# xiaohong-huang/RTK-Visual-Inertial-Navigation

Hardware: AMD Instinct MI355X
Metric: gauss_newton_iterations_per_sec (higher is better)
Workload: dtype f64; 1 GPU; BASELINE cfg4: batch of 512 independent cfg3 windows (20 keyframes, 300 features, 3000 observations, 19 IMU factors, 10 satellites x 20 epochs carrier-phase+pseudorange, gauge prior) over the job, 8 dogleg iterations per solve; windows=512, windows_rank0=512

## Files before the change

### rtk_visual_inertial_navigation_amd/build.py

```python
import os
import subprocess

HERE = os.path.dirname(os.path.abspath(__file__))
CSRC = os.path.join(HERE, "csrc")
LIB = os.path.join(HERE, "libswf_hip.so")
SOURCES = ["swf_engine.hip", "swf_plan.cpp", "swf_problem.cpp", "swf_producers.hip", "swf_gnss_epochs.cpp", "swf_lambda.hip", "swf_features.hip", "swf_fixprior.hip", "swf_phasescreen.hip", "swf_gnssepoch.hip", "swf_ddselect.hip"]
HEADERS = ["swf_dev.h", "swf_records.h", "swf_plan.h", "swf_kernels.h", "swf_lmschur.h", "swf_chol_rr4.h", "swf_kernels2.h", "swf_kernels3.h", "swf_rootdev.h", "swf_kernels4.h", "swf_lambda.h", "swf_features.h", "swf_fixprior.h", "swf_gnss_range.h", "swf_phasescreen.h", "swf_gnssepoch.h", "swf_ddselect.h",
           os.path.join("..", "..", "include", "swf_types.h"),
           os.path.join("..", "..", "include", "swf_solver.h")]


def hipcc():
    for p in (os.environ.get("HIPCC"), "/opt/rocm/bin/hipcc", "hipcc"):
        if p and (os.path.isabs(p) and os.path.exists(p) or not os.path.isabs(p)):
            return p
    return "hipcc"


def needs_build():
    if not os.path.exists(LIB):
        return True
    t = os.path.getmtime(LIB)
    for f in SOURCES + HEADERS:
        p = os.path.join(CSRC, f)
        if os.path.exists(p) and os.path.getmtime(p) > t:
            return True
    return False


def build(force=False, verbose=False):
    if not force and not needs_build():
        return LIB
    srcs = [os.path.join(CSRC, s) for s in SOURCES if os.path.exists(os.path.join(CSRC, s))]
    cmd = [hipcc(), "--offload-arch=gfx950", "-O3", "-std=c++17", "-fPIC", "-shared"] + \
        os.environ.get("SWF_EXTRA_FLAGS", "").split() + ["-x", "hip", "-o", LIB] + srcs
    if verbose:
        print(" ".join(cmd))
    subprocess.check_call(cmd, cwd=CSRC)
    return LIB


if __name__ == "__main__":
    print(build(force=True, verbose=True))
```

### rtk_visual_inertial_navigation_amd/csrc/swf_engine.hip

```cpp
#include <hip/hip_runtime.h>
#include <algorithm>
#include <chrono>
#include <cmath>
#include <cstdio>
#include <cstdlib>
#include <cstring>
#include <string>
#include <memory>
#include <thread>
#include <vector>
#include "../../include/swf_solver.h"
#include "swf_kernels2.h"
#include "swf_kernels3.h"
#include "swf_kernels4.h"
#include "swf_lambda.h"
#include "swf_ddselect.h"
#include "swf_features.h"
#include "swf_fixprior.h"
#include "swf_plan.h"

static thread_local std::string g_err;
static int fail(int code, const std::string& msg) { g_err = msg; return code; }
#define HIPCHK(x) do { hipError_t e_ = (x); if (e_ != hipSuccess) return fail(SWF_E_NODEVICE, std::string(#x) + ": " + hipGetErrorString(e_)); } while (0)

// ... 155 lines not shown
    DevPool pool;
    hipStream_t stream = nullptr;
    std::vector<WinRec> win;
    std::vector<HostWin> hw;
    int max_tiles = 0, max_prior_dim = 0, max_red = 0, min_red = 1 << 30, n_cu = 256;
    bool clc_imu[5] = { false, false, false, false, false };
    CompArgs CA{}; CompMeta CM{}; int n_comp = 0, comp_nmax = 0, comp_nmin = 1 << 30; long long comp_ne = 0;
    bool comp_eigen_root = false;
    void* h_sum = nullptr; size_t h_sum_bytes = 0;
    double* h_x = nullptr;
    double* co_pose0 = nullptr; double* co_sb0 = nullptr;
    int* mg_tail = nullptr; double* mg_A = nullptr; double* mg_b = nullptr; double* mg_J = nullptr; double* mg_r0 = nullptr; double* mg_w = nullptr; int* mg_rank = nullptr; double* mg_M = nullptr;
    bool mg_valid = false; int mg_ld = 0;
    bool mg_host = false; std::vector<double> h_mgA, h_mgJ, h_mgb, h_mgr0, h_mgw; std::vector<int> h_mgrank;
    double* mg_resM = nullptr; double* mg_resb = nullptr; int* mg_resok = nullptr;
    int* mg_rot = nullptr; int* mg_bjok = nullptr; unsigned long long* mg_crit = nullptr;
    int* tc_tail = nullptr; double* tc_A = nullptr; double* tc_Q = nullptr; double* tc_X = nullptr; int* tc_rank = nullptr; bool tc_valid = false; int tc_ld = 0;
    int* am_first = nullptr; int4* am_pairs = nullptr; double* am_rec = nullptr; int am_rec_ld = 0;
    bool am_valid = false, am_host = false; std::vector<double> h_am;
    std::vector<int> am_nb;
    std::vector<int> am_h_first; std::vector<int4> am_h_pairs;
    int* dd_pairs = nullptr; int* dd_counts = nullptr; int* dd_npair = nullptr;
    char* dd_in = nullptr; char* dd_out = nullptr; size_t dd_in_cap = 0, dd_out_cap = 0; int dd_ne = 0, dd_no = 0;
    std::vector<char> dd_h_in, dd_h_out; std::vector<int> dd_h_pairs, dd_h_counts;
    bool dd_valid = false, dd_host = false;
    const int* dd_tail = nullptr;
    bool am_selected = false, am_sel_host = false;
    FixWin* fx_win = nullptr; int* fx_tailcol = nullptr; double* fx_A = nullptr; double* fx_b = nullptr; double* fx_J = nullptr; double* fx_r0 = nullptr;
    double* fx_eig = nullptr; double* fx_x0 = nullptr; int* fx_rank = nullptr; int* fx_applied = nullptr; int fx_ldn = 0, fx_ldx = 0;
    bool fx_valid = false, fx_host = false; FixPriorArgs fx_args{};
    std::vector<FixWin> fx_h_win; std::vector<int> fx_h_tailcol, fx_sel;
    std::vector<double> h_fxA, h_fxb, h_fxJ, h_fxr0, h_fxeig, h_fxx0; std::vector<int> h_fxrank, h_fxapplied;
    bool fc_built = false, fc_valid = false, fc_host = false; FeatArgs fc{}; char* fc_out = nullptr; size_t fc_bytes = 0; int fc_nfeat = 0;
    std::vector<int> fc_feat0; std::vector<char> h_fc;
    hipStream_t aux = nullptr; hipEvent_t ev_fork[3] = { nullptr, nullptr, nullptr };
    ~swf_batch() {
        if (aux) { (void)hipStreamSynchronize(aux); handle_cache().give(aux); }
        for (auto& e : ev_fork) handle_cache().give(e, false);
    }
    WinState* ws_primary = nullptr; WinState* ws_alt = nullptr; WinState* ws_alt2 = nullptr;
    bool no_decide_fuse = false;
    bool no_step_fuse = false;
    int n_pch_split = 0;
    bool no_spec = false;
    bool no_comp_fuse = false;
    bool lat_fuse = false;
    bool rr4_has15 = false, rr4_has16 = false;
    int rr_nmax = 256;
    bool L_full = false;
    int asm_programs = 0;
    int ls_qpb = 1, ls_var = 0, ls_kms = 8; bool ls_folded = false, s_direct = false;
    bool full_final = false;
    bool no_clq_pack = false;
    int clp_rows = 1, clp_ld = 3;
    int ls_gqpb = 4;
    int timing = 0;
    swf_timing last{};
    std::vector<hipEvent_t> ev;
    std::vector<int> ev_kind;
    int ev_used = 0;
    int64_t jac_bytes = 0, proj_bytes = 0, chol_flops = 0, lm_schur_flops = 0, lm_schur_flops_sym = 0, lm_schur_mfma = 0;
    int last_mode = -1;
};

extern "C" int swf_batch_create(const swf_flat_window* const* windows, int32_t n, void* stream, swf_batch** out) {
    if (!windows || n <= 0 || !out) return fail(SWF_E_INVALID, "swf_batch_create: bad arguments");
    int ndev = 0;
    if (hipGetDeviceCount(&ndev) != hipSuccess || ndev <= 0)
        return fail(SWF_E_NODEVICE, "no HIP device: this library has no CPU fallback");
    int n_cu = 256;
    { int dev = 0; hipDeviceProp_t pr; if (hipGetDevice(&dev) == hipSuccess && hipGetDeviceProperties(&pr, dev) == hipSuccess && pr.multiProcessorCount > 0) n_cu = pr.multiProcessorCount; }
    Plan B;
    {
        std::string err;
        int prc = plan_build(windows, n, plan_shape_from_env(n_cu), B, err);
        if (prc != SWF_OK) return fail(prc, err);
    }
    std::unique_ptr<swf_batch> owner(new swf_batch());
    swf_batch* b = owner.get();
    b->device = current_device();
    b->stream = (hipStream_t)stream;
    b->n_cu = n_cu;
    b->no_comp_fuse = getenv("SWF_NO_COMP_FUSE") != nullptr;
    b->no_spec = getenv("SWF_NO_SPEC_EVAL") != nullptr;
    b->no_step_fuse = getenv("SWF_NO_STEP_FUSE") != nullptr;
    b->no_decide_fuse = getenv("SWF_NO_DECIDE_FUSE") != nullptr;
    b->full_final = getenv("SWF_FULL_FINAL_ELIM") != nullptr;
    b->no_clq_pack = getenv("SWF_NO_CLIQUE_PACK") != nullptr;
    b->max_tiles = B.max_tiles; b->max_prior_dim = B.max_prior_dim; b->max_red = B.max_red; b->min_red = B.min_red;
    b->rr_nmax = B.rr_nmax; b->rr4_has15 = B.rr4_has15; b->rr4_has16 = B.rr4_has16; b->n_pch_split = B.n_pch_split;
    b->lat_fuse = B.lat_fuse; b->asm_programs = B.asm_programs;
    b->ls_qpb = B.ls_qpb; b->ls_var = B.ls_var; b->ls_kms = B.ls_kms; b->ls_gqpb = B.ls_gqpb; b->ls_folded = B.ls_folded; b->s_direct = B.s_direct;
    for (int k = 0; k < 5; k++) b->clc_imu[k] = B.clc_imu[k];
    b->clp_rows = B.clp_rows; b->clp_ld = B.clp_ld;
    b->n_comp = B.n_comp; b->comp_nmax = B.comp_nmax; b->comp_nmin = B.comp_nmin; b->comp_ne = B.comp_ne;
    b->jac_bytes = B.jac_bytes; b->proj_bytes = B.proj_bytes; b->chol_flops = B.chol_flops;
    b->lm_schur_flops = B.lm_schur_flops; b->lm_schur_flops_sym = B.lm_schur_flops_sym; b->lm_schur_mfma = B.lm_schur_mfma;
    if (B.want_aux) {
        bool ok = (b->aux = handle_cache().stream()) != nullptr;
        for (int i = 0; i < 3 && ok; i++) ok = (b->ev_fork[i] = handle_cache().event(false)) != nullptr;
        if (!ok) { handle_cache().give(b->aux); b->aux = nullptr; }
    }
    DevBatch& D = b->D;
    DevPool& P = b->pool;
    int rc = 0;
    D.n_win = n; D.n_x = (int)B.n_x; D.n_loc_total = (int)B.n_loc; D.max_iter_trace = SWF_MAX_TRACE; D.rr_nmax = B.rr_nmax;
    D.n_lmb = B.n_lmb; D.n_pch = B.n_pch; D.n_proj = B.n_proj; D.n_lm = B.n_lm; D.n_fr = B.n_fr; D.n_fsb = B.n_fsb;
    D.n_gf = (int)B.gf.size(); D.n_imu = (int)B.imu_gf.size(); D.n_sc = (int)B.sc_gf.size(); D.n_prior = (int)B.prior_gf.size(); D.n_idp = (int)B.idp_gf.size();
    D.n_cl = (int)B.cl.size(); D.n_pair = (int)B.pair.size(); D.n_pd = B.n_pd; D.n_po = B.n_po; D.n_cle = B.n_cle;
    for (int k = 0; k < 5; k++) D.n_clc[k] = B.n_clc[k];
    D.as_max_ne = B.as_max_ne; D.as_max_nv = B.as_max_nv;
#define PUT(field) rc |= P.put(B.field, &D.field)
    PUT(win);
    PUT(lmb_rec); PUT(pch_q); PUT(pch_r0); PUT(prior_nch);
    PUT(blk_xoff); PUT(blk_loc); PUT(blk_gs);
    PUT(loc2x); PUT(x_var);
    PUT(p_win); PUT(p_xpose); PUT(p_xex); PUT(p_xlm);
    PUT(p_lpose); PUT(p_llm); PUT(p_fr); PUT(p_lm); PUT(p_uv);
    PUT(lm_win); PUT(lm_obs0); PUT(lm_loc); PUT(lm_col); PUT(lm_fmask);
    PUT(sch_c0); PUT(sch_rec); PUT(sch_km);
    PUT(fr_obs0); PUT(fr_obs); PUT(fr_red);
    PUT(fsb_rec);
    PUT(fsb_perm); PUT(fsb_foff);
    PUT(gf);
    PUT(s_x); PUT(s_loc); PUT(s_ls); PUT(s_joff); PUT(s_ccol);
    PUT(imu_pre); PUT(cp_dat); PUT(pr_dat); PUT(dop_dat); PUT(sp_w); PUT(gx_dat);
    PUT(imu_gf); PUT(sc_gf); PUT(prior_gf); PUT(idp_gf);
    PUT(sc_jt); PUT(imu_jt);
    PUT(prior_dim); PUT(prior_Joff); PUT(prior_roff); PUT(prior_x0off);
    PUT(prior_Jt);
    PUT(prior_colloc); PUT(prior_colcc); PUT(s_pcol); PUT(s_pxo);
    PUT(prior_J); PUT(prior_r0); PUT(prior_x0);
    PUT(cl); PUT(cl_fac); PUT(cl_frow); PUT(cm_loc); PUT(cm_ls); PUT(cm_col);
    PUT(cv_loc);
    PUT(pc_coff); PUT(pc_cld); PUT(pc_voff);
    PUT(asw); PUT(s_tnz);
    PUT(as_dst); PUT(as_cnt); PUT(as_src0); PUT(as_aux); PUT(as_src);
    PUT(av_loc); PUT(av_red); PUT(av_cnt); PUT(av_src0); PUT(av_i); PUT(av_src);
    PUT(pair_d); PUT(pair_o);
    PUT(cle_rec);
    for (int k = 0; k < 5; k++) PUT(clc_rec[k]);
// ... 303 lines not shown
        hipStream_t sa = fork ? b->aux : st;
        if (fork) { (void)hipEventRecord(b->ev_fork[0], st); (void)hipStreamWaitEvent(b->aux, b->ev_fork[0], 0); }
        bool imu_fused = false;
        if (D.n_proj + D.n_sc + D.n_prior) {
            Bracket t(*this, SWF_K_EVAL_PS);
            bool pf = b->max_prior_dim <= PRIOR_LDS_DIM;
            Segs S{}; S.e[0] = D.n_fsb; S.e[1] = S.e[0] + nb(D.n_sc, 256); S.e[2] = S.e[1] + (pf ? D.n_pch : 0);
            imu_fused = b->lat_fuse && D.n_imu > 0;
            S.e[3] = S.e[2] + (imu_fused ? nb(D.n_imu, IMU_FPB) : 0);
            if (imu_fused) hipLaunchKernelGGL((k_eval_ps<true, true, true>), dim3(S.e[3]), dim3(256), 0, st, D, S);
            else hipLaunchKernelGGL((k_eval_ps<true, true>), dim3(S.e[2]), dim3(256), 0, st, D, S);
        }
        if (D.n_idp) hipLaunchKernelGGL(k_eval_idp<true>, GRID(D.n_idp, 128), dim3(128), 0, st, D);
        if (D.n_prior && b->max_prior_dim > PRIOR_LDS_DIM) { Bracket t(*this, SWF_K_EVAL_PRIOR); hipLaunchKernelGGL(k_eval_prior<true>, dim3(D.n_pch), dim3(256), (2 * b->max_prior_dim + 16) * sizeof(double), st, D); }
        if (fork) (void)hipEventRecord(b->ev_fork[1], st);
        if (D.n_imu && !imu_fused) { Bracket t(*this, SWF_K_EVAL_IMU, sa); hipLaunchKernelGGL(k_eval_imu<true>, GRID(D.n_imu, IMU_FPB), dim3(IMU_FPB * IMU_LPF), 0, sa, D); }
    }
    void lin_elim(int write_S) {
        DevBatch& D = b->D;
        bool clq_fused = false;
        if (comp_fused) {
            Bracket t(*this, SWF_K_CLIQUE_ELIM);
            if (D.n_clc[3]) {
                hipLaunchKernelGGL(k_clique_big2, dim3(D.n_clc[3] + D.n_clc[2]), dim3(CB_NT), 0, st, D, O);
                if (D.n_clc[4]) hipLaunchKernelGGL(k_clique_tall<false>, dim3(D.n_clc[4]), dim3(256), 0, st, D, O);
            } else if (D.n_clc[4] + D.n_clc[2]) hipLaunchKernelGGL(k_clique_tall2, dim3(D.n_clc[4] + D.n_clc[2]), dim3(256), 0, st, D, O);
        } else if (D.n_lm) {
            Bracket t(*this, write_S ? SWF_K_LM_SCHUR : SWF_K_LM_ELIM);
            lm_qpb = b->ls_qpb; lm_folded = b->ls_folded;
            if (!write_S && !b->full_final) {
                dim3 grid(D.n_win, GEMM_SPLIT / b->ls_gqpb);
                hipLaunchKernelGGL((k_lm_schur<8, 2, 2, 80, false, true>), grid, dim3(256), 0, st, D, O, b->ls_gqpb, 0, 0, 0);
            } else if (!write_S) {
                dim3 grid(D.n_win, GEMM_SPLIT / lm_qpb);
                hipLaunchKernelGGL((k_lm_schur<8, 2, 2, 80, false>), grid, dim3(256), 0, st, D, O, lm_qpb, 0, 0, 0);
            } else {
                const int crow = D.n_win > 0 ? (D.n_clc[2] + D.n_win - 1) / D.n_win : 0;
                clq_fused = clq_fuse_ok();
                lm_launch(0, st, clq_fused ? crow : 0);
                lm_next = ls_tiles_per_launch();
            }
        }
        {
            hipStream_t sa = b->aux ? b->aux : st;
            if (b->aux) (void)hipStreamWaitEvent(b->aux, b->ev_fork[1], 0);
            auto cstream = [&](int cls) { return (b->aux && !b->clc_imu[cls]) ? st : sa; };
            if (comp_fused) {
                for (; lm_next < b->max_tiles; lm_next += ls_tiles_per_launch()) { Bracket t(*this, SWF_K_LM_SCHUR, sa); lm_launch(lm_next, sa); }
            } else {
            const bool grad = !write_S && !b->full_final;
            if (D.n_clc[1]) {
                Bracket t(*this, SWF_K_CLIQUE_ELIM, cstream(1));
                if (grad) hipLaunchKernelGGL((k_clique_elim<32, 48, 9, 1, true>), dim3(D.n_clc[1]), dim3(64), 0, cstream(1), D, O);
                else hipLaunchKernelGGL((k_clique_elim<32, 48, 9, 1>), dim3(D.n_clc[1]), dim3(64), 0, cstream(1), D, O);
            }
            if (D.n_clc[0]) {
                Bracket t(*this, SWF_K_CLIQUE_ELIM, cstream(0));
                constexpr int CLP_NW = 1;
                const size_t lds = CLP_NW * 2 * ((size_t)(b->clp_rows + 2) * b->clp_ld + b->clp_rows + 2) * sizeof(double);
                const dim3 cgrid(((D.n_clc[0] + 1) / 2 + CLP_NW - 1) / CLP_NW);
                if (b->no_clq_pack) {
                    if (grad) hipLaunchKernelGGL((k_clique_elim<48, 32, 1, 0, true>), dim3(D.n_clc[0]), dim3(64), 0, cstream(0), D, O);
                    else hipLaunchKernelGGL((k_clique_elim<48, 32, 1, 0>), dim3(D.n_clc[0]), dim3(64), 0, cstream(0), D, O);
                }
                else if (grad) hipLaunchKernelGGL((k_clique_pack<true, CLP_NW>), cgrid, dim3(64 * CLP_NW), lds, cstream(0), D, O, b->clp_rows, b->clp_ld);
                else hipLaunchKernelGGL((k_clique_pack<false, CLP_NW>), cgrid, dim3(64 * CLP_NW), lds, cstream(0), D, O, b->clp_rows, b->clp_ld);
            }
            if (D.n_clc[2] && !clq_fused) {
                Bracket t(*this, SWF_K_CLIQUE_ELIM, cstream(2));
                if (b->lat_fuse) {
                    if (grad) hipLaunchKernelGGL(k_clique_elim4<true>, dim3(D.n_clc[2]), dim3(256), 0, cstream(2), D, O);
                    else hipLaunchKernelGGL(k_clique_elim4<false>, dim3(D.n_clc[2]), dim3(256), 0, cstream(2), D, O);
                }
                else if (grad) hipLaunchKernelGGL((k_clique_elim<64, 64, 9, 2, true>), dim3(D.n_clc[2]), dim3(64), 0, cstream(2), D, O);
                else hipLaunchKernelGGL((k_clique_elim<64, 64, 9, 2>), dim3(D.n_clc[2]), dim3(64), 0, cstream(2), D, O);
            }
            if (D.n_clc[3]) { Bracket t(*this, SWF_K_CLIQUE_ELIM, cstream(3)); hipLaunchKernelGGL(k_clique_big, dim3(D.n_clc[3]), dim3(CB_NT), 0, cstream(3), D, O); }
            if (D.n_clc[4]) {
                Bracket t(*this, SWF_K_CLIQUE_ELIM, cstream(4));
                if (grad) hipLaunchKernelGGL(k_clique_tall<true>, dim3(D.n_clc[4]), dim3(256), 0, cstream(4), D, O);
                else hipLaunchKernelGGL(k_clique_tall<false>, dim3(D.n_clc[4]), dim3(256), 0, cstream(4), D, O);
            }
            if (write_S && D.n_lm) {
                for (; lm_next < b->max_tiles; lm_next += ls_tiles_per_launch()) { Bracket t(*this, SWF_K_LM_SCHUR, sa); lm_launch(lm_next, sa); }
            }
            }
            if (b->aux) (void)hipEventRecord(b->ev_fork[2], b->aux);
        }
        if (b->n_pch_split) hipLaunchKernelGGL(k_prior_graw, dim3(D.n_pch), dim3(256), 0, st, D);
        if (b->aux) (void)hipStreamWaitEvent(st, b->ev_fork[2], 0);
        if (D.n_pd) {
            Bracket t(*this, SWF_K_ASSEMBLE);
            const int nbS = write_S ? nb((size_t)D.as_max_ne, 256) : 0, nbV = nb((size_t)D.as_max_nv, 256);
            hipLaunchKernelGGL(k_assemble_flat, dim3(nbS + nbV, D.n_win), dim3(256), 0, st, D, O, write_S, nbS);
        }
    }
    void reduced() {
        DevBatch& D = b->D;
        Bracket t(*this, SWF_K_CHOL);
        if (b->max_red <= CB_NMAX) {
            if (b->min_red <= b->rr_nmax) {
                if (b->min_red <= 224) hipLaunchKernelGGL(k_chol_rr4<14>, dim3(D.n_win), dim3(R4_NT), 0, st, D, export_full ? 1 : 0);
                if (b->rr4_has15) hipLaunchKernelGGL(k_chol_rr4<15>, dim3(D.n_win), dim3(R4_NT), 0, st, D, export_full ? 1 : 0);
                if (b->rr4_has16) hipLaunchKernelGGL(k_chol_rr4<16>, dim3(D.n_win), dim3(R4_NT), 0, st, D, export_full ? 1 : 0);
            }
            if (b->max_red > b->rr_nmax && D.Wk) {
                const int Tc = (b->max_red + 15) / 16;
// ... 911 lines not shown
        if (r) ok &= dl(r + row, D.g_r + G.roff, (size_t)G.nres * 8);
        if (J && G.type == GF_PRIOR) {
            int dim = 0; long long jo = 0;
            ok &= dl(&dim, D.prior_dim + G.data, 4); ok &= dl(&jo, D.prior_Joff + G.data, 8);
            std::vector<double> PJ((size_t)dim * dim);
            ok &= dl(PJ.data(), D.prior_J + jo, PJ.size() * 8);
            for (int sl = 0; sl < G.nslot; sl++) {
                if (sloc[sl] < 0) continue;
                for (int k = 0; k < G.nres; k++) for (int c = 0; c < sls[sl]; c++)
                    J[(row + k) * nl + (sloc[sl] - W.loc_base) + c] = PJ[(size_t)k * dim + spc[sl] + c];
            }
        } else if (J) {
            for (int sl = 0; sl < G.nslot; sl++) {
                if (sloc[sl] < 0 || sj[sl] < 0) continue;
                std::vector<double> blk((size_t)sls[sl] * G.jld);
                ok &= dl(blk.data(), D.g_J + sj[sl], (((size_t)sls[sl] - 1) * G.jld + G.nres) * 8);
                for (int k = 0; k < G.nres; k++) for (int c = 0; c < sls[sl]; c++)
                    J[(row + k) * nl + (sloc[sl] - W.loc_base) + c] = blk[(size_t)c * G.jld + k];
            }
        }
        if (G.type != GF_PROJX) row_seq += G.nres;
    }
    if (!ok) return fail(SWF_E_NODEVICE, "download failed");
    return SWF_OK;
}

extern "C" int swf_debug_plan_check(const swf_flat_window* const* windows, int32_t n, int32_t n_cu, int32_t ls_variant, int32_t ls_qpb, int32_t ls_grad_qpb,
                                    int32_t flags, int32_t corrupt_table, int32_t corrupt_index, int32_t* info) {
    if (!windows || n <= 0 || n_cu <= 0) return fail(SWF_E_INVALID, "swf_debug_plan_check: bad arguments");
    PlanShape sh;
    sh.n_cu = n_cu; sh.ls_variant = ls_variant; sh.ls_qpb = ls_qpb; sh.ls_grad_qpb = ls_grad_qpb; sh.no_lat_fuse = flags & 1; sh.no_chol_col = flags & 2;
    Plan B; std::string err;
    int rc = plan_build(windows, n, sh, B, err);
    if (rc != SWF_OK) return fail(rc, err);
    if (corrupt_table) {
        const size_t i = (size_t)corrupt_index;
        if (corrupt_table == 1 && i < B.as_src.size()) B.as_src[i] += 1 << 28;
        else if (corrupt_table == 2 && i < B.sch_rec.size()) B.sch_rec[i] ^= 1;
        else if (corrupt_table == 3 && i < B.s_tnz.size() && B.s_tnz[i]) B.s_tnz[i] &= B.s_tnz[i] - 1;
        else if (corrupt_table == 4 && i < B.prior_colloc.size()) B.prior_colloc[i] ^= 1;
        else if (corrupt_table == 5 && i < B.loc2x.size()) B.loc2x[i] ^= 1;
        else if (corrupt_table == 6 && i < B.co_voff.size()) B.co_voff[i] += 1 << 28;
        else if (corrupt_table == 7 && i < B.pair_o.size()) B.pair_o[i].q_base += 8;
        else return fail(SWF_E_INVALID, "swf_debug_plan_check: nothing to corrupt there");
    }
    if (info) {
        const int v[12] = { B.ls_var, B.ls_qpb, B.ls_gqpb, B.ls_folded, B.lat_fuse, B.want_aux, B.want_Linv, B.want_Wk, B.asm_programs, B.n_pch_split, B.max_red, B.n_pch };
        for (int k = 0; k < 12; k++) info[k] = v[k];
    }
    rc = plan_validate(B, err);
    return rc == SWF_OK ? SWF_OK : fail(rc, err);
}

#ifdef SWF_PROFILE_CHOL
extern "C" int swf_debug_chol_stamps(unsigned long long* out) {
    if (hipDeviceSynchronize() != hipSuccess) return SWF_E_NODEVICE;
    if (hipMemcpyFromSymbol(out, HIP_SYMBOL(g_chol_stamps), 64 * sizeof(unsigned long long)) != hipSuccess) return SWF_E_NODEVICE;
    return SWF_OK;
}
#endif

#ifdef SWF_PROFILE_CHOLW
extern "C" int swf_debug_chol_wstep(int step) {
    if (hipDeviceSynchronize() != hipSuccess) return SWF_E_NODEVICE;
    unsigned long long z[16 * 8] = { 0 };
    if (hipMemcpyToSymbol(HIP_SYMBOL(g_chol_wst), z, sizeof(z)) != hipSuccess) return SWF_E_NODEVICE;
    if (hipMemcpyToSymbol(HIP_SYMBOL(g_chol_wstep), &step, sizeof(int)) != hipSuccess) return SWF_E_NODEVICE;
    return SWF_OK;
}
extern "C" int swf_debug_chol_wstamps(unsigned long long* out) {
    if (hipDeviceSynchronize() != hipSuccess) return SWF_E_NODEVICE;
    if (hipMemcpyFromSymbol(out, HIP_SYMBOL(g_chol_wst), 16 * 8 * sizeof(unsigned long long)) != hipSuccess) return SWF_E_NODEVICE;
    return SWF_OK;
}
extern "C" int swf_debug_chol_pstamps(unsigned long long* out) {
    if (hipDeviceSynchronize() != hipSuccess) return SWF_E_NODEVICE;
    if (hipMemcpyFromSymbol(out, HIP_SYMBOL(g_chol_pst), 16 * sizeof(unsigned long long)) != hipSuccess) return SWF_E_NODEVICE;
    return SWF_OK;
}
extern "C" int swf_debug_chol_cstamps(unsigned long long* out) {
    if (hipDeviceSynchronize() != hipSuccess) return SWF_E_NODEVICE;
    if (hipMemcpyFromSymbol(out, HIP_SYMBOL(g_chol_cst), 32 * sizeof(unsigned long long)) != hipSuccess) return SWF_E_NODEVICE;
    return SWF_OK;
}
#endif

#ifdef SWF_PROFILE_DOG
extern "C" int swf_debug_dog_stamps(unsigned long long* out) {
    if (hipDeviceSynchronize() != hipSuccess) return SWF_E_NODEVICE;
    if (hipMemcpyFromSymbol(out, HIP_SYMBOL(g_dog_stamps), 16 * sizeof(unsigned long long)) != hipSuccess) return SWF_E_NODEVICE;
    return SWF_OK;
}
#endif

#ifdef SWF_PROFILE_CLQ
extern "C" int swf_debug_clq_stamps(unsigned long long* out) {
    if (hipDeviceSynchronize() != hipSuccess) return SWF_E_NODEVICE;
    if (hipMemcpyFromSymbol(out, HIP_SYMBOL(g_clq_stamps), 16 * sizeof(unsigned long long)) != hipSuccess) return SWF_E_NODEVICE;
    return SWF_OK;
}
#endif

#ifdef SWF_PROFILE_EVAL
extern "C" int swf_debug_eval_stamps(unsigned long long* out) {
    if (hipDeviceSynchronize() != hipSuccess) return SWF_E_NODEVICE;
    if (hipMemcpyFromSymbol(out, HIP_SYMBOL(g_eval_stamps), 16 * sizeof(unsigned long long)) != hipSuccess) return SWF_E_NODEVICE;
// ... 143 lines not shown
```

### rtk_visual_inertial_navigation_amd/csrc/swf_kernels.h

```cpp
#pragma once
#include "swf_dev.h"

struct DevOpt {
    int max_iter, step_mode, strategy, jacobi;
    double r0, max_r, min_r, min_rel_dec, ftol, gtol, ptol, min_mu, max_mu, mu_inc, min_diag, max_diag;
};



__device__ __forceinline__ double damp_diag(const DevOpt& O, double d, double* jsc_slot, bool first) {
    if (!O.jacobi) return clampd(d, O.min_diag, O.max_diag);
    double q;
    if (first) { double r = 1.0 + sqrt(d > 0.0 ? d : 0.0); q = r * r; *jsc_slot = q; }
    else q = *jsc_slot;
    return clampd(d / q, O.min_diag, O.max_diag) * q;
}

template <bool JAC> __device__ __forceinline__ bool eval_gate(const DevBatch& B, const WinState& s) { return B.spec == 2 ? true : (JAC && !B.spec) ? s.need_lin != 0 : s.eval_cand != 0; }
template <bool JAC> __device__ __forceinline__ const double* eval_src(const DevBatch& B) { return (JAC && !B.spec) ? B.x : B.xc; }

#include "swf_gnss_range.h"

template <bool JAC, bool STORE>
__device__ __forceinline__ double proj_core(const DevBatch& B, int i, const WinRec& W, const double* P, const double* E, const double* X,
// ... 1013 lines not shown
        int nb = (df + 1) >> 1, nblk = nb * (nb + 1) / 2;
        for (int t0 = tid; t0 < nblk; t0 += 2 * NT) {
            int i0[2], j0[2];
            bool diag[2], on[2];
#pragma unroll
            for (int u = 0; u < 2; u++) {
                int t = t0 + NT * u;
                on[u] = t < nblk;
                if (!on[u]) t = 0;
                int ba = (int)((sqrtf(8.0f * t + 1.0f) - 1.0f) * 0.5f);
                while ((ba + 1) * (ba + 2) / 2 <= t) ba++;
                while (ba * (ba + 1) / 2 > t) ba--;
                int bb = t - ba * (ba + 1) / 2;
                i0[u] = 2 * ba; j0[u] = 2 * bb; diag[u] = ba == bb;
            }
            double m[2][4] = { { 0, 0, 0, 0 }, { 0, 0, 0, 0 } };
#pragma unroll UK
            for (int k = 0; k < nrow; k++) {
#pragma unroll
                for (int u = 0; u < 2; u++) {
                    double xa0 = Jc[k][de + i0[u]], xa1 = Jc[k][de + i0[u] + 1], xb0 = Jc[k][de + j0[u]], xb1 = Jc[k][de + j0[u] + 1];
                    m[u][0] += xa0 * xb0; m[u][1] += xa0 * xb1; m[u][2] += xa1 * xb0; m[u][3] += xa1 * xb1;
                }
            }
#pragma unroll(NW > 1 ? 1 : MAXE)
            for (int a2 = 0; a2 < (NW > 1 ? de : MAXE); a2++) {
#pragma unroll
                for (int u = 0; u < 2; u++) {
                    double f0 = Me[a2][de + i0[u]], f1 = Me[a2][de + i0[u] + 1], t0_ = T[a2][j0[u]], t1_ = T[a2][j0[u] + 1];
                    m[u][0] -= f0 * t0_; m[u][1] -= f0 * t1_; m[u][2] -= f1 * t0_; m[u][3] -= f1 * t1_;
                }
            }
#pragma unroll
            for (int u = 0; u < 2; u++) {
                if (!on[u]) continue;
                int i = i0[u], j = j0[u];
                bool i1ok = i + 1 < df, j1ok = j + 1 < df;
                Cm[i * df + j] = m[u][0]; Cm[j * df + i] = m[u][0];
                if (i1ok) { Cm[(i + 1) * df + j] = m[u][2]; Cm[j * df + i + 1] = m[u][2]; }
                if (!diag[u] && j1ok) { Cm[i * df + j + 1] = m[u][1]; Cm[(j + 1) * df + i] = m[u][1]; }
                if (i1ok && j1ok) { Cm[(i + 1) * df + j + 1] = m[u][3]; Cm[(j + 1) * df + i + 1] = m[u][3]; }
            }
        }
    }
    QST(5);
}
template <int MAXR, int MAXD, int MAXE, int CLS, bool GRAD = false>
__global__ void __launch_bounds__(64) k_clique_elim(DevBatch B, DevOpt O) { d_clique_elim<MAXR, MAXD, MAXE, CLS, 24, 1, 4, GRAD>(B, O, (int)blockIdx.x); }
template <bool GRAD = false>
__global__ void __launch_bounds__(256) k_clique_elim4(DevBatch B, DevOpt O) { d_clique_elim<64, 64, 9, 2, 8, 4, 4, GRAD>(B, O, (int)blockIdx.x); }
template <bool GRAD = false>
__global__ void __launch_bounds__(256) k_clique_tall(DevBatch B, DevOpt O) { d_clique_elim<CLQ_TALLR, 64, 9, 4, 8, 4, 4, GRAD>(B, O, (int)blockIdx.x); }

__device__ __forceinline__ double readhalf_d(double v, bool upper) { double a = readlane_d(v, 0), b = readlane_d(v, 32); return upper ? b : a; }
template <bool GRAD, int NW>
__global__ void __launch_bounds__(64 * NW) k_clique_pack(DevBatch B, DevOpt O, const int R, const int LD) {
    constexpr int PF = 12;
    extern __shared__ double clp_lds[];
    const int lane = threadIdx.x & 63, hl = lane & 31, pair = (int)blockIdx.x * NW + (NW > 1 ? __builtin_amdgcn_readfirstlane((int)threadIdx.x >> 6) : 0);
    const bool up = lane >= 32;
    double* Jc = clp_lds + (2 * (pair - (int)blockIdx.x * NW) + (up ? 1 : 0)) * ((R + 2) * LD + R + 2);
    double* rv = Jc + R * LD; double* Me = rv + R; double* T = Me + LD; double* Ei = T + LD; double* Eg = Ei + 1;
    const int n = B.n_clc[0];
    int cidx = 2 * pair + (up ? 1 : 0);
    bool act = cidx < n;
    const Clique& C = B.clc_rec[0][act ? cidx : 0];
    WinState& s = B.ws[C.win];
    act = act && s.need_lin;
    if (__builtin_amdgcn_ballot_w64(act) == 0) return;
    const int de = act ? C.d_e : 0, df = act ? C.d_f : 0, d = de + df, nrow = act ? C.n_rows : 0, tot = nrow * d;
    const int nrow_m = max(__builtin_amdgcn_readlane(nrow, 0), __builtin_amdgcn_readlane(nrow, 32));
    const int tot_m = max(__builtin_amdgcn_readlane(tot, 0), __builtin_amdgcn_readlane(tot, 32));
    {
        const double* gJ = B.g_J + C.j_off;
        float rd = 1.0f / (float)(nrow > 0 ? nrow : 1);
        const double r0 = hl < nrow ? B.g_r[C.r_off + hl] : 0.0, r1 = hl + 32 < nrow ? B.g_r[C.r_off + hl + 32] : 0.0;
        for (int k = hl; k < nrow; k += 32) { Jc[k * LD + d] = 0.0; Jc[k * LD + d + 1] = 0.0; }
        for (int base = 0; base < tot_m; base += PF * 32) {
            double v[PF];
#pragma unroll
            for (int u = 0; u < PF; u++) { int e = base + u * 32 + hl; v[u] = e < tot ? gJ[e] : 0.0; }
#pragma unroll
            for (int u = 0; u < PF; u++) {
                int e = base + u * 32 + hl;
                int col = (int)((e + 0.5f) * rd);
                col += (e - col * nrow >= nrow) ? 1 : 0; col -= (e - col * nrow < 0) ? 1 : 0;
                if (e < tot) Jc[(e - col * nrow) * LD + col] = v[u];
            }
        }
        if (hl < nrow) rv[hl] = r0;
        if (hl + 32 < nrow) rv[hl + 32] = r1;
    }
    __builtin_amdgcn_fence(__ATOMIC_SEQ_CST, "workgroup");
    __builtin_amdgcn_wave_barrier();
    double me = 0, gc = 0, mcc = 0;
    {
        const int c = hl < d ? hl : 0;
#pragma unroll 4
        for (int k = 0; k < nrow_m; k++) {
            if (k < nrow) {
                double x = Jc[k * LD + c];
                gc += x * rv[k]; mcc += x * x;
                if (!GRAD) me += Jc[k * LD] * x;
            }
        }
    }
// ... 381 lines not shown
```

Before: 716,700 iterations/s.

## Use f64 MFMA for class-1 clique elimination Gram and Schur products

Adds a new clique elimination kernel for class-1 cliques that forms J^T J and the Schur update -Me^T T with 16x16x4 f64 MFMA instructions over three 16-column tiles. It replaces the scalar per-lane products of the existing k_clique_elim on the non-gradient path, and the old kernel stays reachable through an environment variable. The intent is to cut FMA work in this per-clique stage. In exchange it adds zero padding, extra LDS traffic and MFMA fragment layout handling, and it only covers one clique class with a single wave per block. A small debug kernel and host entry point for checking the MFMA layout are also added.

```diff
diff --git a/rtk_visual_inertial_navigation_amd/build.py b/rtk_visual_inertial_navigation_amd/build.py
--- a/rtk_visual_inertial_navigation_amd/build.py
+++ b/rtk_visual_inertial_navigation_amd/build.py
@@ -5,7 +5,7 @@
 CSRC = os.path.join(HERE, "csrc")
 LIB = os.path.join(HERE, "libswf_hip.so")
 SOURCES = ["swf_engine.hip", "swf_plan.cpp", "swf_problem.cpp", "swf_producers.hip", "swf_gnss_epochs.cpp", "swf_lambda.hip", "swf_features.hip", "swf_fixprior.hip", "swf_phasescreen.hip", "swf_gnssepoch.hip", "swf_ddselect.hip"]
-HEADERS = ["swf_dev.h", "swf_records.h", "swf_plan.h", "swf_kernels.h", "swf_lmschur.h", "swf_chol_rr4.h", "swf_kernels2.h", "swf_kernels3.h", "swf_rootdev.h", "swf_kernels4.h", "swf_lambda.h", "swf_features.h", "swf_fixprior.h", "swf_gnss_range.h", "swf_phasescreen.h", "swf_gnssepoch.h", "swf_ddselect.h",
+HEADERS = ["swf_dev.h", "swf_records.h", "swf_plan.h", "swf_kernels.h", "swf_clique_mm.h", "swf_lmschur.h", "swf_chol_rr4.h", "swf_kernels2.h", "swf_kernels3.h", "swf_rootdev.h", "swf_kernels4.h", "swf_lambda.h", "swf_features.h", "swf_fixprior.h", "swf_gnss_range.h", "swf_phasescreen.h", "swf_gnssepoch.h", "swf_ddselect.h",
            os.path.join("..", "..", "include", "swf_types.h"),
            os.path.join("..", "..", "include", "swf_solver.h")]
 
diff --git a/rtk_visual_inertial_navigation_amd/csrc/swf_clique_mm.h b/rtk_visual_inertial_navigation_amd/csrc/swf_clique_mm.h
--- /dev/null
+++ b/rtk_visual_inertial_navigation_amd/csrc/swf_clique_mm.h
@@ -0,0 +1,206 @@
+#pragma once
+
+__device__ constexpr int CMM_SLOT_ROW[4] = { 0, 1, 2, 3 };
+
+__global__ void __launch_bounds__(64) k_debug_mfma_f64(const double* A, const double* Bm, const double* Cm, double* Dm) {
+    const int lane = threadIdx.x, i = lane & 15, k = lane >> 4;
+    double4_t c;
+#pragma unroll
+    for (int r = 0; r < 4; r++) c[r] = Cm[(k + 4 * r) * 16 + i];
+    c = __builtin_amdgcn_mfma_f64_16x16x4f64(A[i * 4 + k], Bm[k * 16 + i], c, 0, 0, 0);
+#pragma unroll
+    for (int r = 0; r < 4; r++) Dm[(k + 4 * r) * 16 + i] = c[r];
+}
+
+template <int MAXR, int MAXD, int MAXE>
+__global__ void __launch_bounds__(64) k_clique_mm(DevBatch B, DevOpt O) {
+    static_assert(MAXR % 4 == 0 && MAXD == 48 && MAXE <= 16, "k_clique_mm: whole k-steps, three 16-column tiles, the eliminated block inside tile column 0");
+    constexpr int LD = MAXD + 1, CLS = 1, PF = 24, KE = (MAXE + 3) / 4;
+    __shared__ double lds[MAXR * LD + MAXR];
+    static_assert((2 * MAXD + MAXE + 1) * MAXE <= MAXR * LD, "k_clique_mm: Me | T | Ei | Eg inside the Jacobian's storage");
+    double (*Jc)[LD] = reinterpret_cast<double (*)[LD]>(lds);
+    double* rv = lds + MAXR * LD;
+    double (*Me)[MAXD] = reinterpret_cast<double (*)[MAXD]>(lds);
+    double (*T)[MAXD] = reinterpret_cast<double (*)[MAXD]>(lds + MAXE * MAXD);
+    double (*Ei)[MAXE] = reinterpret_cast<double (*)[MAXE]>(lds + 2 * MAXE * MAXD);
+    double* Eg = lds + 2 * MAXE * MAXD + MAXE * MAXE;
+    const int cidx_ = (int)blockIdx.x;
+#ifdef SWF_PROFILE_CLQ
+    unsigned long long tq_ = __builtin_amdgcn_s_memtime();
+    if (cidx_ == SWF_PROFILE_CLQ_IDX && threadIdx.x == 0) for (int i = 0; i < 16; i++) g_clq_stamps[i] = 0;
+#endif
+    if (cidx_ >= B.n_clc[CLS]) return;
+    const Clique& C = B.clc_rec[CLS][cidx_];
+    WinState& s = B.ws[C.win];
+    if (!s.need_lin) return;
+    const int lane = threadIdx.x, li = lane & 15, lk = lane >> 4;
+    const int de = C.d_e, df = C.d_f, d = de + df, nrow = C.n_rows, nr4 = (nrow + 3) & ~3;
+    const int nt = (d + 15) >> 4;
+    QST(0);
+    {
+        const double* gJ = B.g_J + C.j_off;
+        int tot = nrow * d;
+        float rd = 1.0f / (float)nrow;
+        if (lane < nrow) rv[lane] = B.g_r[C.r_off + lane];
+        for (int e = lane; e < (nr4 - nrow) * MAXD; e += 64) Jc[nrow + e / MAXD][e % MAXD] = 0.0;
+        for (int e = lane; e < nrow * (MAXD - d); e += 64) Jc[e % nrow][d + e / nrow] = 0.0;
+        for (int base = 0; base < tot; base += PF * 64) {
+            double v[PF];
+#pragma unroll
+            for (int u = 0; u < PF; u++) { int e = base + u * 64 + lane; v[u] = e < tot ? gJ[e] : 0.0; }
+#pragma unroll
+            for (int u = 0; u < PF; u++) {
+                int e = base + u * 64 + lane;
+                int col = (int)((e + 0.5f) * rd);
+                col += (e - col * nrow >= nrow) ? 1 : 0; col -= (e - col * nrow < 0) ? 1 : 0;
+                if (e < tot) Jc[e - col * nrow][col] = v[u];
+            }
+        }
+    }
+    __syncthreads();
+    QST(1);
+    double4_t acc[6];
+#pragma unroll
+    for (int t = 0; t < 6; t++) acc[t] = double4_t{ 0, 0, 0, 0 };
+    for (int k0 = 0; k0 < nr4; k0 += 4) {
+        const int k = k0 + CMM_SLOT_ROW[lk];
+        double x[3];
+#pragma unroll
+        for (int t = 0; t < 3; t++) x[t] = t < nt ? Jc[k][16 * t + li] : 0.0;
+#pragma unroll
+        for (int ti = 0; ti < 3; ti++)
+#pragma unroll
+            for (int tj = 0; tj <= ti; tj++)
+                if (ti < nt) acc[ti * (ti + 1) / 2 + tj] = __builtin_amdgcn_mfma_f64_16x16x4f64(x[ti], x[tj], acc[ti * (ti + 1) / 2 + tj], 0, 0, 0);
+    }
+    double gc = 0;
+    {
+        const int c = lane < d ? lane : 0;
+#pragma unroll 4
+        for (int k = 0; k < nrow; k++) gc += Jc[k][c] * rv[k];
+    }
+    __syncthreads();
+#pragma unroll
+    for (int ti = 0; ti < 3; ti++) {
+        if (ti < nt) {
+#pragma unroll
+            for (int r = 0; r < 4; r++) {
+                const int row = lk + 4 * r;
+                if (row == li) T[0][16 * ti + li] = acc[ti * (ti + 1) / 2 + ti][r];
+                if (li < MAXE) Me[li][16 * ti + row] = li < de ? acc[ti * (ti + 1) / 2][r] : 0.0;
+            }
+        }
+    }
+    __syncthreads();
+    if (lane < d) {
+        const double mcc = T[0][lane];
+        if (lane < de) { B.g[C.e_loc + lane] = gc; B.diag[C.e_loc + lane] = mcc; B.vc[C.e_loc + lane] = gc / clampd(mcc, O.min_diag, O.max_diag); }
+        else { B.cv_graw[C.v_off + lane - de] = gc; B.cv_dgraw[C.v_off + lane - de] = mcc; }
+    }
+    __syncthreads();
+    QST(2);
+    if (de > 0) {
+        {
+            double row[2 * MAXE];
+#pragma unroll
+            for (int j = 0; j < MAXE; j++) {
+                double v = (lane < de && j < de) ? Me[lane][j] : 0.0;
+                if (j == lane) v += s.mu * (lane < de ? damp_diag(O, v, B.jsc + C.e_loc + lane, s.iter == 0) : clampd(v, O.min_diag, O.max_diag));
+                row[j] = v; row[MAXE + j] = (j == lane) ? 1.0 : 0.0;
+            }
+            bool bad = false;
+#pragma unroll
+            for (int k = 0; k < MAXE; k++) {
+                if (k < de) {
+                    double piv = readlane_d(row[k], k);
+                    if (!(piv > 0.0)) bad = true;
+                    double ip = __builtin_amdgcn_rcp(piv);
+                    ip = ip * (2.0 - piv * ip); ip = ip * (2.0 - piv * ip);
+                    double aik = row[k];
+#pragma unroll
+                    for (int j = 0; j < 2 * MAXE; j++) {
+                        double akj = readlane_d(row[j], k) * ip;
+                        row[j] = (lane == k) ? akj : row[j] - aik * akj;
+                    }
+                }
+            }
+            if (bad) { if (lane == 0) s.lin_fail = 1; return; }
+            if (lane < MAXE) {
+#pragma unroll
+                for (int j = 0; j < MAXE; j++) Ei[lane][j] = (lane < de && j < de) ? row[MAXE + j] : 0.0;
+            }
+        }
+        __syncthreads();
+        QST(3);
+        {
+            double gE = 0;
+            int j = lane < df ? lane : 0;
+            double mcol[MAXE], gb[MAXE];
+#pragma unroll
+            for (int b2 = 0; b2 < MAXE; b2++) { mcol[b2] = Me[b2][de + j]; gb[b2] = readlane_d(gc, b2); }
+#pragma unroll 1
+            for (int a2 = 0; a2 < MAXE; a2++) {
+                double sv = 0, sg = 0;
+#pragma unroll
+                for (int b2 = 0; b2 < MAXE; b2++) { double ev = Ei[a2][b2]; sv += ev * mcol[b2]; sg += ev * gb[b2]; }
+                if (lane < df) T[a2][lane] = sv;
+                if (lane == a2) gE = sg;
+            }
+            if (lane < de) Eg[lane] = gE;
+        }
+        __syncthreads();
+        QST(4);
+        double* E = B.cE + C.e_off;
+        {
+            for (int e = lane; e < de * de; e += 64) E[e] = Ei[e / de][e % de];
+            if (lane < df) {
+#pragma unroll
+                for (int a2 = 0; a2 < MAXE; a2++) if (a2 < de) E[de * de + a2 * df + lane] = Me[a2][de + lane];
+            }
+            if (lane < de) E[de * de + de * df + lane] = gc;
+            if (lane < df) {
+                double v = 0;
+#pragma unroll
+                for (int a2 = 0; a2 < MAXE; a2++) v -= Me[a2][de + lane] * (a2 < de ? Eg[a2] : 0.0);
+                B.cv_cs[C.v_off + lane] = v;
+            }
+        }
+#pragma unroll
+        for (int ks = 0; ks < KE; ks++) {
+            const int a2 = 4 * ks + CMM_SLOT_ROW[lk], a2c = a2 < MAXE ? a2 : 0;
+            double fa[3], tb[3];
+#pragma unroll
+            for (int t = 0; t < 3; t++) {
+                const int cc = 16 * t + li - de;
+                const bool on = t < nt && a2 < MAXE;
+                fa[t] = on ? -Me[a2c][16 * t + li] : 0.0;
+                tb[t] = on && cc >= 0 && cc < df ? T[a2c][cc] : 0.0;
+            }
+#pragma unroll
+            for (int ti = 0; ti < 3; ti++)
+#pragma unroll
+                for (int tj = 0; tj <= ti; tj++)
+                    if (ti < nt) acc[ti * (ti + 1) / 2 + tj] = __builtin_amdgcn_mfma_f64_16x16x4f64(fa[ti], tb[tj], acc[ti * (ti + 1) / 2 + tj], 0, 0, 0);
+        }
+    } else {
+        if (lane < df) B.cv_cs[C.v_off + lane] = 0.0;
+    }
+    double* Cm = B.C + C.C_off;
+#pragma unroll
+    for (int ti = 0; ti < 3; ti++)
+#pragma unroll
+        for (int tj = 0; tj <= ti; tj++) {
+            if (ti < nt) {
+#pragma unroll
+                for (int r = 0; r < 4; r++) {
+                    const int R = 16 * ti + lk + 4 * r, Cc = 16 * tj + li;
+                    if (R >= Cc && Cc >= de && R < d) {
+                        const int i = R - de, j = Cc - de;
+                        const double v = acc[ti * (ti + 1) / 2 + tj][r];
+                        Cm[i * df + j] = v; Cm[j * df + i] = v;
+                    }
+                }
+            }
+        }
+    QST(5);
+}
diff --git a/rtk_visual_inertial_navigation_amd/csrc/swf_engine.hip b/rtk_visual_inertial_navigation_amd/csrc/swf_engine.hip
--- a/rtk_visual_inertial_navigation_amd/csrc/swf_engine.hip
+++ b/rtk_visual_inertial_navigation_amd/csrc/swf_engine.hip
@@ -231,6 +231,7 @@
     int ls_qpb = 1, ls_var = 0, ls_kms = 8; bool ls_folded = false, s_direct = false;
     bool full_final = false;
     bool no_clq_pack = false;
+    bool no_clq_mfma = false;
     int clp_rows = 1, clp_ld = 3;
     int ls_gqpb = 4;
     int timing = 0;
@@ -266,6 +267,7 @@
     b->no_decide_fuse = getenv("SWF_NO_DECIDE_FUSE") != nullptr;
     b->full_final = getenv("SWF_FULL_FINAL_ELIM") != nullptr;
     b->no_clq_pack = getenv("SWF_NO_CLIQUE_PACK") != nullptr;
+    b->no_clq_mfma = getenv("SWF_NO_CLIQUE_MFMA") != nullptr;
     b->max_tiles = B.max_tiles; b->max_prior_dim = B.max_prior_dim; b->max_red = B.max_red; b->min_red = B.min_red;
     b->rr_nmax = B.rr_nmax; b->rr4_has15 = B.rr4_has15; b->rr4_has16 = B.rr4_has16; b->n_pch_split = B.n_pch_split;
     b->lat_fuse = B.lat_fuse; b->asm_programs = B.asm_programs;
@@ -675,7 +677,8 @@
             if (D.n_clc[1]) {
                 Bracket t(*this, SWF_K_CLIQUE_ELIM, cstream(1));
                 if (grad) hipLaunchKernelGGL((k_clique_elim<32, 48, 9, 1, true>), dim3(D.n_clc[1]), dim3(64), 0, cstream(1), D, O);
-                else hipLaunchKernelGGL((k_clique_elim<32, 48, 9, 1>), dim3(D.n_clc[1]), dim3(64), 0, cstream(1), D, O);
+                else if (b->no_clq_mfma) hipLaunchKernelGGL((k_clique_elim<32, 48, 9, 1>), dim3(D.n_clc[1]), dim3(64), 0, cstream(1), D, O);
+                else hipLaunchKernelGGL((k_clique_mm<32, 48, 9>), dim3(D.n_clc[1]), dim3(64), 0, cstream(1), D, O);
             }
             if (D.n_clc[0]) {
                 Bracket t(*this, SWF_K_CLIQUE_ELIM, cstream(0));
@@ -1693,6 +1696,21 @@
     return rc == SWF_OK ? SWF_OK : fail(rc, err);
 }
 
+extern "C" int swf_debug_mfma_f64(const double* A, const double* Bm, const double* C, double* D) {
+    if (!A || !Bm || !C || !D) return fail(SWF_E_INVALID, "swf_debug_mfma_f64: bad arguments");
+    double* dv = nullptr;
+    if (hipMalloc(&dv, (64 + 64 + 256 + 256) * sizeof(double)) != hipSuccess) return fail(SWF_E_NODEVICE, "swf_debug_mfma_f64: allocation failed");
+    bool ok = hipMemcpy(dv, A, 64 * sizeof(double), hipMemcpyHostToDevice) == hipSuccess
+        && hipMemcpy(dv + 64, Bm, 64 * sizeof(double), hipMemcpyHostToDevice) == hipSuccess
+        && hipMemcpy(dv + 128, C, 256 * sizeof(double), hipMemcpyHostToDevice) == hipSuccess;
+    if (ok) {
+        hipLaunchKernelGGL(k_debug_mfma_f64, dim3(1), dim3(64), 0, 0, dv, dv + 64, dv + 128, dv + 384);
+        ok = hipGetLastError() == hipSuccess && hipMemcpy(D, dv + 384, 256 * sizeof(double), hipMemcpyDeviceToHost) == hipSuccess;
+    }
+    (void)hipFree(dv);
+    return ok ? SWF_OK : fail(SWF_E_NODEVICE, "swf_debug_mfma_f64: the device run failed");
+}
+
 #ifdef SWF_PROFILE_CHOL
 extern "C" int swf_debug_chol_stamps(unsigned long long* out) {
     if (hipDeviceSynchronize() != hipSuccess) return SWF_E_NODEVICE;
diff --git a/rtk_visual_inertial_navigation_amd/csrc/swf_kernels.h b/rtk_visual_inertial_navigation_amd/csrc/swf_kernels.h
--- a/rtk_visual_inertial_navigation_amd/csrc/swf_kernels.h
+++ b/rtk_visual_inertial_navigation_amd/csrc/swf_kernels.h
@@ -1089,6 +1089,8 @@
 template <bool GRAD = false>
 __global__ void __launch_bounds__(256) k_clique_tall(DevBatch B, DevOpt O) { d_clique_elim<CLQ_TALLR, 64, 9, 4, 8, 4, 4, GRAD>(B, O, (int)blockIdx.x); }
 
+#include "swf_clique_mm.h"
+
 __device__ __forceinline__ double readhalf_d(double v, bool upper) { double a = readlane_d(v, 0), b = readlane_d(v, 32); return upper ? b : a; }
 template <bool GRAD, int NW>
 __global__ void __launch_bounds__(64 * NW) k_clique_pack(DevBatch B, DevOpt O, const int R, const int LD) {
```

New measurement: 727,400 iterations/s, median of 6. 1.5% higher.
